# LarsELund/Bayesian-Neural-Nets

Measured on AMD Instinct MI355X. Metric: ELBO forward samples/sec, 784-1200^2-10 MNF MLP, batch 4096 per GPU, higher is better.
Workload: dtype f16 (row-scaled fp16 hi + lo split of the f32 operands: 3 mean + 1 variance MFMA products, f32 accumulate)

## Files before the change

bayesian-neural-nets_amd/csrc/gemm_common.h:

```cpp
#pragma once
#include <cstdlib>
#include <hip/hip_runtime.h>
#include <stdint.h>

namespace {

__device__ __forceinline__ void tile_of_block(int& ox, int& by, int extra_rows = 0) {
    const int nx = gridDim.x, ny = gridDim.y - extra_rows, n = nx * ny;
    int t = blockIdx.y * nx + blockIdx.x;
    if ((n & 7) == 0 && (ny & 3) == 0) {
        const int xcd = t & 7, s = t >> 3, per = n >> 3, q = ny >> 2;
        const int idx = (xcd & 1) * per + s;
        ox = idx / q;
        by = (xcd >> 1) * q + idx % q;
        return;
    }
    if ((n & 7) == 0) t = (t & 7) * (n >> 3) + (t >> 3);
    ox = t % nx; by = t / nx;
}

constexpr size_t kLdsPerCU = 160 * 1024;
constexpr int kNumCU = 256;

inline size_t lds_request(size_t needed, long nblocks) {
    long r = (nblocks + kNumCU - 1) / kNumCU;
    static const char* const res_env = getenv("LBBNN_GEMM_RESIDENCY");
    if (res_env) r = atol(res_env);
    if (r < 1) r = 1;
    if (r >= 3) return needed;
    const size_t cap = kLdsPerCU / (size_t)(r + 1) + 256;
    return needed > cap ? needed : cap;
}

template <typename K, typename A>
inline int launch_one(K kernel, dim3 grid, dim3 block, size_t lds, hipStream_t s, const A& a) {
    if (lds > 64 * 1024) {
        static size_t raised = 0;
        if (lds > raised) {
            hipError_t e = hipFuncSetAttribute(reinterpret_cast<const void*>(kernel),
                                               hipFuncAttributeMaxDynamicSharedMemorySize, (int)lds);
            if (e != hipSuccess) return (int)e;
            raised = lds;
        }
    }
    hipLaunchKernelGGL(kernel, grid, block, lds, s, a);
    return (int)hipGetLastError();
}


}
```

bayesian-neural-nets_amd/csrc/lrt_gemm_f16.hip:

```cpp
#include <cstdlib>
#include "lbbnn_device.h"
#include "lbbnn_internal.h"
#include "kl_piggy.h"
#include "gemm_common.h"
#include "../../include/lbbnn.h"

namespace {

using namespace lbbnn;
typedef float floatx4 __attribute__((ext_vector_type(4)));
typedef float floatx2 __attribute__((ext_vector_type(2)));
typedef _Float16 f16x8 __attribute__((ext_vector_type(8)));
typedef _Float16 f16x2 __attribute__((ext_vector_type(2)));

constexpr int BKS = 32;
constexpr float kS2 = 0.00390625f;
constexpr float kS2inv = 256.f;

__device__ __forceinline__ int swzx(int r) { return (((r >> 1) & 3) << 1) | ((r >> 3) & 1); }
__device__ __forceinline__ int swz4(int rowgrp) { return (0x78 >> (2 * (rowgrp & 3))) & 3; }

struct G16Args {
    const char* x; const char* e_w; const char* var_w;
    const float* mean_scale; const float* wvar_scale;
    const float* bias_mean; const float* bias_var; const float* var_scale;
    const float* eps; const uint64_t* rng;
    float* out; char* out_planes; float* std_out;
    long long row_offset;
    int ldx, ld, ldo, ldp, B, I, O;
    uint32_t rng_stream;
    int relu;
    const float* h_e; const float* h_v; float* h_slab;
    int h_ld, h_C;
    FinalizePiggy fin;
};

typedef _Float16 f16x4 __attribute__((ext_vector_type(4)));
constexpr float kHeadES = 256.f, kHeadVS = 16384.f;

__device__ __forceinline__ uint32_t cvt_pk_h(float a, float b) {
    const floatx2 v = {a, b};
    return __builtin_bit_cast(uint32_t, __builtin_convertvector(v, f16x2));
}
__device__ __forceinline__ float h_lo(uint32_t p) { return (float)__builtin_bit_cast(f16x2, p)[0]; }
__device__ __forceinline__ float h_hi(uint32_t p) { return (float)__builtin_bit_cast(f16x2, p)[1]; }

struct OC16 { float bm[4], bv[4], vs[4], ms[4]; };

__device__ __forceinline__ void ld4f(const float* p, int o, int O, float fill, float out[4]) {
    if (!p) { out[0] = out[1] = out[2] = out[3] = fill; return; }
    if (o + 3 < O && ((reinterpret_cast<uintptr_t>(p + o) & 15u) == 0)) {
        const float4 t = *reinterpret_cast<const float4*>(p + o);
        out[0] = t.x; out[1] = t.y; out[2] = t.z; out[3] = t.w;
    } else {
#pragma unroll
        for (int r = 0; r < 4; ++r) out[r] = (o + r < O) ? p[o + r] : fill;
    }
}

template <int TO, int TB, int NPV>
__device__ __forceinline__ void epilogue16(const G16Args& a, int o0, int q, int lr, int brow0,
                                           const floatx4 (&accm)[TO][TB], const floatx4 (&accv)[TO][TB]) {
    const bool ovec = ((a.O & 3) == 0) && (!a.out || (((a.ldo & 3) == 0) && ((reinterpret_cast<uintptr_t>(a.out) & 15u) == 0))) &&
                      (!a.eps || (reinterpret_cast<uintptr_t>(a.eps) & 15u) == 0) &&
                      (!a.std_out || (reinterpret_cast<uintptr_t>(a.std_out) & 15u) == 0);
    uint64_t seed = 0, offs = 0;
    if (!a.eps) { seed = a.rng[0]; offs = a.rng[1]; }
    OC16 oc[TO];
#pragma unroll
    for (int i = 0; i < TO; ++i) {
        const int o = o0 + i * 16 + 4 * q;
        if (o < a.O) {
            ld4f(a.bias_mean, o, a.O, 0.f, oc[i].bm);
            ld4f(a.bias_var, o, a.O, 0.f, oc[i].bv);
            ld4f(a.var_scale, o, a.O, 1.f, oc[i].vs);
            ld4f(a.mean_scale, o, a.O, 1.f, oc[i].ms);
            float wv[4];
            ld4f(a.wvar_scale, o, a.O, 1.f, wv);
#pragma unroll
            for (int r = 0; r < 4; ++r) oc[i].vs[r] = (wv[r] * kS2inv) * oc[i].vs[r];
        }
    }
    float pe[TO][TB][4];
    if (a.eps) {
#pragma unroll
        for (int i = 0; i < TO; ++i) {
            const int o = o0 + i * 16 + 4 * q;
#pragma unroll
            for (int j = 0; j < TB; ++j) {
                const int b = brow0 + j * 16;
                if (o >= a.O || b >= a.B) continue;
                const float* p = a.eps + (size_t)b * a.O + o;
                if (ovec) { const float4 t = *reinterpret_cast<const float4*>(p); pe[i][j][0] = t.x; pe[i][j][1] = t.y; pe[i][j][2] = t.z; pe[i][j][3] = t.w; }
                else {
#pragma unroll
                    for (int r = 0; r < 4; ++r) pe[i][j][r] = (o + r < a.O) ? p[r] : 0.f;
                }
            }
        }
    }
    const bool head = a.h_slab != nullptr;
    float4 he4[TO], hv4[TO];
    if (head) {
#pragma unroll
        for (int i = 0; i < TO; ++i) {
            const int o = o0 + i * 16 + 4 * q;
            he4[i] = make_float4(0.f, 0.f, 0.f, 0.f); hv4[i] = he4[i];
            if (lr < a.h_C && o < a.O) {
                he4[i] = *reinterpret_cast<const float4*>(a.h_e + (size_t)lr * a.h_ld + o);
                hv4[i] = *reinterpret_cast<const float4*>(a.h_v + (size_t)lr * a.h_ld + o);
            }
        }
    }
    __builtin_amdgcn_sched_barrier(0);
    const bool odd = q & 1;
    floatx4 hm[TB], hv[TB];
#pragma unroll
    for (int j = 0; j < TB; ++j) { hm[j] = floatx4{0.f, 0.f, 0.f, 0.f}; hv[j] = floatx4{0.f, 0.f, 0.f, 0.f}; }
#pragma unroll
    for (int i = 0; i < TO; ++i) {
        const int o = o0 + i * 16 + 4 * q;
        const bool oin = o < a.O;
        f16x4 ehd = {0, 0, 0, 0}, eld = {0, 0, 0, 0}, vhd = {0, 0, 0, 0}, vld = {0, 0, 0, 0};
        if (head) {
            const float4 e4 = he4[i], v4 = hv4[i];
            const uint32_t eh0 = cvt_pk_h(e4.x * kHeadES, e4.y * kHeadES), eh1 = cvt_pk_h(e4.z * kHeadES, e4.w * kHeadES);
            const uint32_t el0 = cvt_pk_h(e4.x * kHeadES - h_lo(eh0), e4.y * kHeadES - h_hi(eh0));
            const uint32_t el1 = cvt_pk_h(e4.z * kHeadES - h_lo(eh1), e4.w * kHeadES - h_hi(eh1));
            const uint32_t vh0 = cvt_pk_h(v4.x * kHeadVS, v4.y * kHeadVS), vh1 = cvt_pk_h(v4.z * kHeadVS, v4.w * kHeadVS);
            ehd = __builtin_bit_cast(f16x4, make_uint2(eh0, eh1)); eld = __builtin_bit_cast(f16x4, make_uint2(el0, el1));
            vhd = __builtin_bit_cast(f16x4, make_uint2(vh0, vh1));
            if (NPV == 3) {
                const uint32_t vl0 = cvt_pk_h(v4.x * kHeadVS - h_lo(vh0), v4.y * kHeadVS - h_hi(vh0));
                const uint32_t vl1 = cvt_pk_h(v4.z * kHeadVS - h_lo(vh1), v4.w * kHeadVS - h_hi(vh1));
                vld = __builtin_bit_cast(f16x4, make_uint2(vl0, vl1));
            }
        }
#pragma unroll
        for (int j = 0; j < TB; ++j) {
            const int b = brow0 + j * 16;
            const bool live = oin && b < a.B;
            float e[4] = {0.f, 0.f, 0.f, 0.f};
            if (a.eps) {
#pragma unroll
                for (int r = 0; r < 4; ++r) e[r] = pe[i][j][r];
            } else if (live) {
                philox_normal4(seed, offs, a.rng_stream, (uint64_t)(a.row_offset + b), (uint32_t)(o >> 2), e);
            }
            float res[4], sd[4];
#pragma unroll
            for (int r = 0; r < 4; ++r) {
                sd[r] = sqrt_hw(accv[i][j][r] * oc[i].vs[r] + oc[i].bv[r]);
                const float m = accm[i][j][r] * oc[i].ms[r] + oc[i].bm[r] + sd[r] * e[r];
                res[r] = a.relu ? fmaxf(m, 0.f) : m;
            }
            if (a.out && live) {
                float* p = a.out + (size_t)b * a.ldo + o;
                if (ovec) *reinterpret_cast<float4*>(p) = make_float4(res[0], res[1], res[2], res[3]);
                else {
#pragma unroll
                    for (int r = 0; r < 4; ++r) if (o + r < a.O) p[r] = res[r];
                }
            }
            if (a.std_out && live) {
                float* p = a.std_out + (size_t)b * a.O + o;
                if (ovec) *reinterpret_cast<float4*>(p) = make_float4(sd[0], sd[1], sd[2], sd[3]);
                else {
#pragma unroll
                    for (int r = 0; r < 4; ++r) if (o + r < a.O) p[r] = sd[r];
                }
            }
            if (head) {
                float hx[4];
#pragma unroll
                for (int r = 0; r < 4; ++r) hx[r] = (live && o + r < a.O) ? res[r] : 0.f;
                const uint32_t h01 = cvt_pk_h(hx[0], hx[1]), h23 = cvt_pk_h(hx[2], hx[3]);
                const uint32_t l01 = cvt_pk_h(hx[0] - h_lo(h01), hx[1] - h_hi(h01)), l23 = cvt_pk_h(hx[2] - h_lo(h23), hx[3] - h_hi(h23));
                const f16x4 xh = __builtin_bit_cast(f16x4, make_uint2(h01, h23)), xl = __builtin_bit_cast(f16x4, make_uint2(l01, l23));
                const float s0 = hx[0] * hx[0] * kS2, s1 = hx[1] * hx[1] * kS2, s2 = hx[2] * hx[2] * kS2, s3 = hx[3] * hx[3] * kS2;
                const uint32_t q01 = cvt_pk_h(s0, s1), q23 = cvt_pk_h(s2, s3);
                const f16x4 sh = __builtin_bit_cast(f16x4, make_uint2(q01, q23));
                hm[j] = __builtin_amdgcn_mfma_f32_16x16x16f16(ehd, xh, hm[j], 0, 0, 0);
                hm[j] = __builtin_amdgcn_mfma_f32_16x16x16f16(eld, xh, hm[j], 0, 0, 0);
                hm[j] = __builtin_amdgcn_mfma_f32_16x16x16f16(ehd, xl, hm[j], 0, 0, 0);
                hv[j] = __builtin_amdgcn_mfma_f32_16x16x16f16(vhd, sh, hv[j], 0, 0, 0);
                if (NPV == 3) {
                    const uint32_t r01 = cvt_pk_h(s0 - h_lo(q01), s1 - h_hi(q01)), r23 = cvt_pk_h(s2 - h_lo(q23), s3 - h_hi(q23));
                    const f16x4 sl = __builtin_bit_cast(f16x4, make_uint2(r01, r23));
                    hv[j] = __builtin_amdgcn_mfma_f32_16x16x16f16(vld, sh, hv[j], 0, 0, 0);
                    hv[j] = __builtin_amdgcn_mfma_f32_16x16x16f16(vhd, sl, hv[j], 0, 0, 0);
                }
            }
            if (a.out_planes) {
                const uint32_t h01 = cvt_pk_h(res[0], res[1]), h23 = cvt_pk_h(res[2], res[3]);
                const uint32_t l01 = cvt_pk_h(res[0] - h_lo(h01), res[1] - h_hi(h01));
                const uint32_t l23 = cvt_pk_h(res[2] - h_lo(h23), res[3] - h_hi(h23));
                const auto s0 = __builtin_amdgcn_permlane16_swap(h01, l01, false, false);
                const auto s1 = __builtin_amdgcn_permlane16_swap(h23, l23, false, false);
                if (live) {
                    const int kk = o & ~7;
                    char* p = a.out_planes + (size_t)b * a.ldp * 4 + (size_t)(kk >> 5) * 128 + ((kk >> 3) & 3) * 32 + (odd ? 16 : 0);
                    *reinterpret_cast<uint4*>(p) = make_uint4(s0[0], s1[0], s0[1], s1[1]);
                }
            }
        }
    }
    if (head) {
        const int ot = o0 / (TO * 16);
#pragma unroll
        for (int j = 0; j < TB; ++j) {
            const int b = brow0 + j * 16;
            if (b < a.B) {
                float* p = a.h_slab + ((size_t)ot * a.B + b) * 32 + 4 * q;
                *reinterpret_cast<float4*>(p) = make_float4(hm[j][0], hm[j][1], hm[j][2], hm[j][3]);
                *reinterpret_cast<float4*>(p + 16) = make_float4(hv[j][0], hv[j][1], hv[j][2], hv[j][3]);
            }
        }
    }
}

template <int TO, int TB, int WB, int NPV, bool XPL>
__device__ __forceinline__ void gemm_f16s_body(const G16Args& a) {
    static_assert(NPV == 1 || NPV == 3, "one or three variance products");
    constexpr int BN = TO * 16, BM = TB * WB * 16;
    constexpr int VROW = NPV == 1 ? 64 : 128;
    constexpr int XB = BM * 128, WRB = BN * 128, VRB = BN * VROW, BUFB = XB + WRB + VRB;
    constexpr int NGX = BM / 8, NGW = BN / 8, NGV = VRB / 1024, NG = NGX + NGW + NGV, NPW = (NG + WB - 1) / WB;
    static_assert(VRB % 1024 == 0, "whole 1-KiB pieces");
    extern __shared__ __attribute__((aligned(16))) char smc[];

    const int tid = threadIdx.x, lane = tid & 63;
    const int wv = __builtin_amdgcn_readfirstlane(tid >> 6);
    const int lr = lane & 15, q = lane >> 4;
    if (a.fin.n > 0 && blockIdx.y == gridDim.y - 1) {
        if (blockIdx.x == 0) kl_finalize_piggy<WB>(kernarg_as<G16Args>()->fin, reinterpret_cast<float*>(smc));
        return;
    }
    int tox, tby;
    tile_of_block(tox, tby, a.fin.n > 0 ? 1 : 0);
    const int o0 = tox * BN, b0 = tby * BM;

    const size_t xsz = XPL ? (size_t)a.B * a.ldx * 4 : ((size_t)(a.B - 1) * a.ldx + a.I) * 4;
    const unsigned xbytes = (unsigned)min((size_t)0x7FFFFFF0u, xsz);
    const unsigned wbytes = (unsigned)min((size_t)0x7FFFFFF0u, (size_t)a.O * a.ld * 4);
    const __amdgpu_buffer_rsrc_t rx = __builtin_amdgcn_make_buffer_rsrc((void*)a.x, 0, (int)xbytes, 0x00020000);
    const __amdgpu_buffer_rsrc_t re = __builtin_amdgcn_make_buffer_rsrc((void*)a.e_w, 0, (int)wbytes, 0x00020000);
    const __amdgpu_buffer_rsrc_t rv = __builtin_amdgcn_make_buffer_rsrc((void*)a.var_w, 0, (int)(NPV == 1 ? wbytes / 2 : wbytes), 0x00020000);
    int gv[NPW], kx[NPW];
#pragma unroll
    for (int u = 0; u < NPW; ++u) {
        const int g = wv + WB * u;
        if (g < NGX) {
            const int row = 8 * g + (lane >> 3);
            const int slot = (lane & 7) ^ swzx(row & 15);
            gv[u] = (int)((size_t)min(b0 + row, a.B - 1) * a.ldx * 4) + 16 * slot;
            kx[u] = XPL ? -1 : 4 * slot;
        } else if (g < NGX + NGW || NPV == 3) {
            const int gw = g - NGX, row = 8 * (gw % NGW) + (lane >> 3);
            const int slot = (lane & 7) ^ swzx(row & 15);
            gv[u] = (int)((size_t)min(o0 + row, a.O - 1) * a.ld * 4) + 16 * slot;
            kx[u] = -1;
        } else {
            const int gw = g - NGX - NGW, row = 16 * gw + (lane >> 2);
            const int slot = (lane & 3) ^ swz4(row >> 2);
            gv[u] = (int)((size_t)min(o0 + row, a.O - 1) * a.ld * 2) + 16 * slot;
            kx[u] = -1;
        }
    }
    const int nsteps = (a.I + BKS - 1) / BKS;
    const bool has_tail = !XPL && (a.I % BKS) != 0;
    int gvt[NPW];
#pragma unroll
    for (int u = 0; u < NPW; ++u)
        gvt[u] = (kx[u] >= 0 && (nsteps - 1) * BKS + kx[u] >= a.I) ? 0x7FFFFFF0 : gv[u];
    auto dma_pieces = [&](int c, char* buf, const int (&va)[NPW]) {
#pragma unroll
        for (int u = 0; u < NPW; ++u) {
            const int g = wv + WB * u;
            if (g < NG) {
                const int loff = g < NGX ? g * 1024 : XB + (g - NGX) * 1024;
                auto* dst = (__attribute__((address_space(3))) void*)(buf + loff);
                if (g < NGX)                 __builtin_amdgcn_raw_ptr_buffer_load_lds(rx, dst, 16, va[u], c * 128, 0, 0);
                else if (g - NGX < NGW)      __builtin_amdgcn_raw_ptr_buffer_load_lds(re, dst, 16, va[u], c * 128, 0, 0);
                else                         __builtin_amdgcn_raw_ptr_buffer_load_lds(rv, dst, 16, va[u], c * VROW, 0, 0);
            }
        }
    };
    auto dma_step = [&](int c, char* buf) {
        if (has_tail && c == nsteps - 1) dma_pieces(c, buf, gvt);
        else dma_pieces(c, buf, gv);
    };

    floatx4 accm[TO][TB], accv[TO][TB];
#pragma unroll
    for (int i = 0; i < TO; ++i)
#pragma unroll
        for (int j = 0; j < TB; ++j) { accm[i][j] = floatx4{0.f, 0.f, 0.f, 0.f}; accv[i][j] = floatx4{0.f, 0.f, 0.f, 0.f}; }

    const int gx = swzx(lr);
    const int xo0 = (wv * TB * 16 + lr) * 128 + 16 * ((2 * q) ^ gx);
    const int xo1 = (wv * TB * 16 + lr) * 128 + 16 * ((2 * q + 1) ^ gx);
    const int woh = XB + lr * 128 + 16 * ((2 * q) ^ gx);
    const int wol = XB + lr * 128 + 16 * ((2 * q + 1) ^ gx);
    const int vo1 = XB + WRB + lr * 64 + 16 * (q ^ swz4(lr >> 2));

    uint4 xu[TB][2];
    uint4 eh[TO], el[TO], vh[TO], vl[TO];
    auto read_frags = [&](const char* cur) {
#pragma unroll
        for (int j = 0; j < TB; ++j) {
            xu[j][0] = *reinterpret_cast<const uint4*>(cur + xo0 + j * 16 * 128);
            xu[j][1] = *reinterpret_cast<const uint4*>(cur + xo1 + j * 16 * 128);
        }
#pragma unroll
        for (int i = 0; i < TO; ++i) {
            eh[i] = *reinterpret_cast<const uint4*>(cur + woh + i * 16 * 128);
            el[i] = *reinterpret_cast<const uint4*>(cur + wol + i * 16 * 128);
            if (NPV == 3) {
                vh[i] = *reinterpret_cast<const uint4*>(cur + WRB + woh + i * 16 * 128);
                vl[i] = *reinterpret_cast<const uint4*>(cur + WRB + wol + i * 16 * 128);
            } else {
                vh[i] = *reinterpret_cast<const uint4*>(cur + vo1 + i * 16 * 64);
            }
        }
    };
    auto mfmas = [&]() {
        f16x8 xh[TB], xl[TB], sh[TB], sl[TB];
#pragma unroll
        for (int j = 0; j < TB; ++j) {
            if (XPL) {
                xh[j] = __builtin_bit_cast(f16x8, xu[j][0]);
                xl[j] = __builtin_bit_cast(f16x8, xu[j][1]);
                if (NPV == 1) {
                    const f16x8 pa = xh[j] * (_Float16)0.0625f, pb = xl[j] * (_Float16)0.125f;
                    const f16x8 t = pa * pb;
                    sh[j] = pa * pa + t;
                } else {
                    uint32_t ph[4], pl[4];
#pragma unroll
                    for (int t = 0; t < 4; ++t) {
                        const float h0 = (float)xh[j][2 * t], h1 = (float)xh[j][2 * t + 1];
                        const float l0 = (float)xl[j][2 * t], l1 = (float)xl[j][2 * t + 1];
                        const float s0 = (h0 * h0 + 2.f * h0 * l0) * kS2, s1 = (h1 * h1 + 2.f * h1 * l1) * kS2;
                        ph[t] = cvt_pk_h(s0, s1);
                        pl[t] = cvt_pk_h(s0 - h_lo(ph[t]), s1 - h_hi(ph[t]));
                    }
                    sh[j] = __builtin_bit_cast(f16x8, make_uint4(ph[0], ph[1], ph[2], ph[3]));
                    sl[j] = __builtin_bit_cast(f16x8, make_uint4(pl[0], pl[1], pl[2], pl[3]));
                }
            } else {
                const float4 f0 = __builtin_bit_cast(float4, xu[j][0]), f1 = __builtin_bit_cast(float4, xu[j][1]);
                const float v[8] = {f0.x, f0.y, f0.z, f0.w, f1.x, f1.y, f1.z, f1.w};
                uint32_t ph[4], pl[4], qh[4] = {0, 0, 0, 0}, ql[4] = {0, 0, 0, 0};
#pragma unroll
                for (int t = 0; t < 4; ++t) {
                    const float v0 = v[2 * t], v1 = v[2 * t + 1];
                    ph[t] = cvt_pk_h(v0, v1);
                    pl[t] = cvt_pk_h(v0 - h_lo(ph[t]), v1 - h_hi(ph[t]));
                    if (NPV == 3) {
                        const float s0 = (v0 * v0) * kS2, s1 = (v1 * v1) * kS2;
                        qh[t] = cvt_pk_h(s0, s1);
                        ql[t] = cvt_pk_h(s0 - h_lo(qh[t]), s1 - h_hi(qh[t]));
                    }
                }
                xh[j] = __builtin_bit_cast(f16x8, make_uint4(ph[0], ph[1], ph[2], ph[3]));
                xl[j] = __builtin_bit_cast(f16x8, make_uint4(pl[0], pl[1], pl[2], pl[3]));
                if (NPV == 1) {
                    const f16x8 pa = xh[j] * (_Float16)0.0625f, pb = xl[j] * (_Float16)0.125f;
                    const f16x8 t2 = pa * pb;
                    sh[j] = pa * pa + t2;
                } else {
                    sh[j] = __builtin_bit_cast(f16x8, make_uint4(qh[0], qh[1], qh[2], qh[3]));
                }
                sl[j] = __builtin_bit_cast(f16x8, make_uint4(ql[0], ql[1], ql[2], ql[3]));
            }
        }
#pragma unroll
        for (int j = 0; j < TB; ++j) {
#pragma unroll
            for (int i = 0; i < TO; ++i) {
                const f16x8 ah = __builtin_bit_cast(f16x8, eh[i]), al = __builtin_bit_cast(f16x8, el[i]);
                accm[i][j] = __builtin_amdgcn_mfma_f32_16x16x32_f16(ah, xh[j], accm[i][j], 0, 0, 0);
                accm[i][j] = __builtin_amdgcn_mfma_f32_16x16x32_f16(al, xh[j], accm[i][j], 0, 0, 0);
                accm[i][j] = __builtin_amdgcn_mfma_f32_16x16x32_f16(ah, xl[j], accm[i][j], 0, 0, 0);
                const f16x8 bh = __builtin_bit_cast(f16x8, vh[i]);
                accv[i][j] = __builtin_amdgcn_mfma_f32_16x16x32_f16(bh, sh[j], accv[i][j], 0, 0, 0);
                if (NPV == 3) {
                    accv[i][j] = __builtin_amdgcn_mfma_f32_16x16x32_f16(__builtin_bit_cast(f16x8, vl[i]), sh[j], accv[i][j], 0, 0, 0);
                    accv[i][j] = __builtin_amdgcn_mfma_f32_16x16x32_f16(bh, sl[j], accv[i][j], 0, 0, 0);
                }
            }
        }
    };

    dma_step(0, smc);
    __syncthreads();
    for (int c = 0; c < nsteps; ++c) {
        read_frags(smc + (c & 1) * BUFB);
        __builtin_amdgcn_sched_barrier(0);
        if (c + 1 < nsteps) dma_step(c + 1, smc + ((c & 1) ^ 1) * BUFB);
        __builtin_amdgcn_sched_barrier(0);
        mfmas();
        __builtin_amdgcn_sched_barrier(0);
        __syncthreads();
    }
    epilogue16<TO, TB, NPV>(a, o0, q, lr, b0 + wv * TB * 16 + lr, accm, accv);
}

template <int TO, int TB, int WB, int NPV, bool XPL>
__global__ __launch_bounds__(WB * 64, 2) void lrt_gemm_f16s_kernel(const G16Args a) {
    gemm_f16s_body<TO, TB, WB, NPV, XPL>(a);
}

template <int TO, int TB, int WB>
int launch16(G16Args& a, int npv, bool xpl, hipStream_t s, bool* hosted) {
    constexpr int BN = TO * 16, BM = TB * WB * 16;
    dim3 grid((a.O + BN - 1) / BN, (a.B + BM - 1) / BM, 1), block(WB * 64);
    const long nblocks = (long)grid.x * grid.y;
    const size_t lds = lds_request(2u * (BM * 128 + BN * 128 + BN * (npv == 1 ? 64 : 128)), nblocks);
    const int fin_n = a.fin.n;
    a.fin.n = 0;
    if (fin_n > 0 && hosted) {
        a.fin.n = fin_n;
        if (piggy_lds_bytes(a.fin) <= lds) { grid.y += 1; *hosted = true; }
        else a.fin.n = 0;
    }
    if (npv == 1) {
        if (xpl) return launch_one(lrt_gemm_f16s_kernel<TO, TB, WB, 1, true>, grid, block, lds, s, a);
        return launch_one(lrt_gemm_f16s_kernel<TO, TB, WB, 1, false>, grid, block, lds, s, a);
    }
    if (xpl) return launch_one(lrt_gemm_f16s_kernel<TO, TB, WB, 3, true>, grid, block, lds, s, a);
    return launch_one(lrt_gemm_f16s_kernel<TO, TB, WB, 3, false>, grid, block, lds, s, a);
}

__global__ __launch_bounds__(256) void format_x_kernel(const FormatJob j) {
    format_x_items(j, (size_t)blockIdx.x * 256 + threadIdx.x, (size_t)gridDim.x * 256);
}

struct HeadFinArgs {
    const float* slab; const float* bias_mean; const float* bias_var; const float* eps; const uint64_t* rng;
    float* out; long long row_offset;
    int n_ot, B, C, ldo, log_softmax; uint32_t rng_stream;
};

__global__ __launch_bounds__(256) void head_finalize_kernel(const HeadFinArgs a) {
    const int t = blockIdx.x * 256 + threadIdx.x, b = t >> 4, q = (t >> 2) & 3, g = t & 3;
    const bool rowok = b < a.B;
    float m[4] = {0.f, 0.f, 0.f, 0.f}, v[4] = {0.f, 0.f, 0.f, 0.f};
    if (rowok) {
        float4 pm[4], pv[4];
#pragma unroll
        for (int k = 0; k < 4; ++k) {
            const int ot = g + 4 * k;
            pm[k] = make_float4(0.f, 0.f, 0.f, 0.f); pv[k] = pm[k];
            if (ot < a.n_ot) {
                const float* p = a.slab + ((size_t)ot * a.B + b) * 32 + 4 * q;
                pm[k] = *reinterpret_cast<const float4*>(p); pv[k] = *reinterpret_cast<const float4*>(p + 16);
            }
        }
        for (int ot = g + 16; ot < a.n_ot; ot += 4) {
            const float* p = a.slab + ((size_t)ot * a.B + b) * 32 + 4 * q;
            const float4 xm = *reinterpret_cast<const float4*>(p), xv = *reinterpret_cast<const float4*>(p + 16);
            pm[0].x += xm.x; pm[0].y += xm.y; pm[0].z += xm.z; pm[0].w += xm.w;
            pv[0].x += xv.x; pv[0].y += xv.y; pv[0].z += xv.z; pv[0].w += xv.w;
        }
        m[0] = (pm[0].x + pm[1].x) + (pm[2].x + pm[3].x); m[1] = (pm[0].y + pm[1].y) + (pm[2].y + pm[3].y);
        m[2] = (pm[0].z + pm[1].z) + (pm[2].z + pm[3].z); m[3] = (pm[0].w + pm[1].w) + (pm[2].w + pm[3].w);
        v[0] = (pv[0].x + pv[1].x) + (pv[2].x + pv[3].x); v[1] = (pv[0].y + pv[1].y) + (pv[2].y + pv[3].y);
        v[2] = (pv[0].z + pv[1].z) + (pv[2].z + pv[3].z); v[3] = (pv[0].w + pv[1].w) + (pv[2].w + pv[3].w);
    }
#pragma unroll
    for (int r = 0; r < 4; ++r) {
        m[r] += dpp_get<0xB1>(m[r]); m[r] += dpp_get<0x4E>(m[r]);
        v[r] += dpp_get<0xB1>(v[r]); v[r] += dpp_get<0x4E>(v[r]);
    }
    float e[4] = {0.f, 0.f, 0.f, 0.f};
    const int c0 = 4 * q;
    if (rowok && c0 < a.C) {
        if (a.eps) {
#pragma unroll
            for (int r = 0; r < 4; ++r) if (c0 + r < a.C) e[r] = a.eps[(size_t)b * a.C + c0 + r];
        } else {
            philox_normal4(a.rng[0], a.rng[1], a.rng_stream, (uint64_t)(a.row_offset + b), (uint32_t)q, e);
        }
    }
    float res[4];
    float mx = -INFINITY;
#pragma unroll
    for (int r = 0; r < 4; ++r) {
        const int c = c0 + r;
        const bool in = rowok && c < a.C;
        const float bm = (in && a.bias_mean) ? a.bias_mean[c] : 0.f, bv = (in && a.bias_var) ? a.bias_var[c] : 0.f;
        const float sd = sqrt_hw(v[r] * (kS2inv / kHeadVS) + bv);
        res[r] = m[r] * (1.f / kHeadES) + bm + sd * e[r];
        if (in) mx = fmaxf(mx, res[r]);
    }
    if (a.log_softmax) {
        mx = fmaxf(mx, dpp_get<0x141>(mx));
        mx = fmaxf(mx, dpp_get<0x140>(mx));
        float se = 0.f;
#pragma unroll
        for (int r = 0; r < 4; ++r) if (rowok && c0 + r < a.C) se += expf(res[r] - mx);
        se += dpp_get<0x141>(se);
        se += dpp_get<0x140>(se);
        const float lse = mx + logf(se);
#pragma unroll
        for (int r = 0; r < 4; ++r) res[r] -= lse;
    }
    if (rowok && g == 0)
#pragma unroll
        for (int r = 0; r < 4; ++r) if (c0 + r < a.C) a.out[(size_t)b * a.ldo + c0 + r] = res[r];
}

}

extern "C" int64_t lbbnn_head_slab_floats(int B, int O) {
    if (B <= 0 || O <= 0) return 0;
    return (int64_t)((O + 79) / 80) * B * 32;
}

extern "C" int lbbnn_format_x(const float* x, int ldx, void* planes, int ldp, int B, int I, void* stream) {
    if (B == 0) return 0;
    if (!x || !planes) return LBBNN_E_NULL;
    if (B < 0 || I <= 0 || ldx < I || ldp < I) return LBBNN_E_SHAPE;
    if ((I & 7) || (ldx & 3) || (ldp & 31) || (reinterpret_cast<uintptr_t>(x) & 15u) || (reinterpret_cast<uintptr_t>(planes) & 15u))
        return LBBNN_E_ALIGN;
    const size_t n = (size_t)B * (ldp >> 3);
    const int blocks = (int)min((size_t)2048, (n + 255) / 256);
    const FormatJob j{x, static_cast<char*>(planes), ldx, ldp, B, I};
    hipLaunchKernelGGL(format_x_kernel, dim3(blocks), dim3(256), 0, static_cast<hipStream_t>(stream), j);
    return (int)hipGetLastError();
}

extern "C" int lbbnn_lrt_gemm_ex(const lbbnn_gemm_desc_t* d, void* stream) {
    if (!d) return LBBNN_E_NULL;
    const int B = d->B, I = d->I, O = d->O, flags = d->flags;
    if (flags & ~(LBBNN_F_RELU | LBBNN_F_F16S | LBBNN_F_VAR1 | LBBNN_F_XPLANES)) return LBBNN_E_FLAGS;
    if (!(flags & LBBNN_F_F16S)) return LBBNN_E_FLAGS;
    if (B == 0 && I > 0 && O > 0 && d->n_layers == 0 && !d->advance) return 0;
    if (!d->x || !d->e_w || !d->var_w || !d->mean_scale || !d->wvar_scale) return LBBNN_E_NULL;
    if (!d->eps && !d->rng) return LBBNN_E_NOISE;
    if (B <= 0 || I <= 0 || O <= 16 || d->ldx < I || (d->out && d->ldo < O)) return LBBNN_E_SHAPE;
    const bool xpl = (flags & LBBNN_F_XPLANES) != 0;
    if (d->ld < I || (d->ld & 31) || (I & 7)) return LBBNN_E_ALIGN;
    if ((I % BKS) != 0 && (d->ld - I) < 8) return LBBNN_E_ALIGN;
    if ((reinterpret_cast<uintptr_t>(d->e_w) | reinterpret_cast<uintptr_t>(d->var_w) | reinterpret_cast<uintptr_t>(d->x)) & 15u) return LBBNN_E_ALIGN;
    if (xpl ? (d->ldx & 31) != 0 : (d->ldx & 3) != 0) return LBBNN_E_ALIGN;
    if (d->out_planes && ((O & 7) || (d->ldp & 31) || d->ldp < O || (reinterpret_cast<uintptr_t>(d->out_planes) & 15u))) return LBBNN_E_ALIGN;
    if ((size_t)B * d->ldx * 4 >= 0x7FFFFFF0u || (size_t)O * d->ld * 4 >= 0x7FFFFFF0u) return LBBNN_E_SHAPE;
    if (d->n_layers < 0 || (d->n_layers > 0 && !d->layers) || (d->advance && !d->rng_live)) return LBBNN_E_NULL;
    const bool head = d->head_out != nullptr;
    if (head) {
        if (!d->head_e || !d->head_v || !d->head_slab) return LBBNN_E_NULL;
        if (d->head_classes <= 0 || d->head_classes > 16 || d->head_ld < O || (d->head_ld & 3) || d->head_ldo < d->head_classes) return LBBNN_E_SHAPE;
        if ((O & 3) || ((reinterpret_cast<uintptr_t>(d->head_e) | reinterpret_cast<uintptr_t>(d->head_v) | reinterpret_cast<uintptr_t>(d->head_slab)) & 15u)) return LBBNN_E_ALIGN;
        if (!d->head_eps && !d->rng) return LBBNN_E_NOISE;
        if (!(flags & LBBNN_F_RELU)) return LBBNN_E_FLAGS;
    } else if (!d->out && !d->out_planes) return LBBNN_E_NULL;

    G16Args a;
    a.x = static_cast<const char*>(d->x); a.e_w = static_cast<const char*>(d->e_w); a.var_w = static_cast<const char*>(d->var_w);
    a.mean_scale = d->mean_scale; a.wvar_scale = d->wvar_scale;
    a.bias_mean = d->bias_mean; a.bias_var = d->bias_var; a.var_scale = d->var_scale;
    a.eps = d->eps; a.rng = d->rng; a.out = d->out; a.out_planes = static_cast<char*>(d->out_planes); a.std_out = d->std_out;
    a.row_offset = d->row_offset; a.ldx = d->ldx; a.ld = d->ld; a.ldo = d->ldo; a.ldp = d->ldp; a.B = B; a.I = I; a.O = O;
    a.rng_stream = d->rng_stream; a.relu = (flags & LBBNN_F_RELU) ? 1 : 0;
    a.h_e = head ? d->head_e : nullptr; a.h_v = head ? d->head_v : nullptr; a.h_slab = head ? d->head_slab : nullptr;
    a.h_ld = d->head_ld; a.h_C = d->head_classes;
    a.fin = FinalizePiggy{};
    const bool want_fin = d->n_layers > 0 || d->advance;
    if (d->n_layers > 0) {
        if (const int rc = fill_finalize_args(d->layers, d->n_layers, d->fin_rng, a.fin.l, a.fin.active)) return rc;
        if (d->kl_total) for (int i = 0; i < d->n_layers; ++i) if (!a.fin.active[i]) return LBBNN_E_NULL;
        a.fin.n = d->n_layers; a.fin.total = d->kl_total;
        a.fin.rng_adv = d->advance ? d->rng_live : nullptr; a.fin.adv = d->advance;
    }
    hipStream_t s = static_cast<hipStream_t>(stream);
    const int npv = (flags & LBBNN_F_VAR1) ? 1 : 3;
    bool hosted = false;
    const long blocks_big = (long)((O + 79) / 80) * ((B + 127) / 128);
    int rc;
    if (blocks_big >= 256 && B >= 96) rc = launch16<5, 2, 4>(a, npv, xpl, s, &hosted);
    else rc = launch16<5, 1, 2>(a, npv, xpl, s, &hosted);
    if (rc) return rc;
    if (head) {
        HeadFinArgs h;
        h.slab = d->head_slab; h.bias_mean = d->head_bias_mean; h.bias_var = d->head_bias_var; h.eps = d->head_eps; h.rng = d->rng;
        h.out = d->head_out; h.row_offset = d->row_offset; h.n_ot = (O + 79) / 80; h.B = B; h.C = d->head_classes; h.ldo = d->head_ldo;
        h.log_softmax = (d->head_flags & LBBNN_F_LOG_SOFTMAX) ? 1 : 0; h.rng_stream = d->head_rng_stream;
        hipLaunchKernelGGL(head_finalize_kernel, dim3((16 * (size_t)B + 255) / 256), dim3(256), 0, s, h);
        rc = (int)hipGetLastError();
        if (rc) return rc;
    }
    if (!want_fin || hosted) return rc;
    if (d->n_layers > 0)
        return launch_kl_finalize_all(a.fin.l, a.fin.active, d->n_layers, d->advance ? d->rng_live : nullptr, d->advance,
                                      d->kl_total, s);
    return lbbnn_rng_advance(d->rng_live, d->advance, stream);
}
```

Measured before the change: 32.40 million.

## Stage epilogue constants in LDS and precompute Philox noise during prologue

The per-feature bias/scale vectors and head fp16 hi/lo splits are now loaded once per block by one thread per feature during the last K-step and written to the idle LDS buffer, instead of every lane redundantly loading and converting them in the epilogue. Several Philox normal draws are computed right after the first DMA issue so they overlap with memory latency rather than sitting on the epilogue's critical path. Grid tile dimensions are passed as kernel arguments. This adds LDS traffic and extra registers held through the main loop for the precomputed noise, which may lower occupancy.

Result: faster. 33.55 million, median of 6 (+3.5%).

```diff
diff --git a/bayesian-neural-nets_amd/csrc/gemm_common.h b/bayesian-neural-nets_amd/csrc/gemm_common.h
--- a/bayesian-neural-nets_amd/csrc/gemm_common.h
+++ b/bayesian-neural-nets_amd/csrc/gemm_common.h
@@ -5,8 +5,8 @@
 
 namespace {
 
-__device__ __forceinline__ void tile_of_block(int& ox, int& by, int extra_rows = 0) {
-    const int nx = gridDim.x, ny = gridDim.y - extra_rows, n = nx * ny;
+__device__ __forceinline__ void tile_of_block(int& ox, int& by, int nx, int ny) {
+    const int n = nx * ny;
     int t = blockIdx.y * nx + blockIdx.x;
     if ((n & 7) == 0 && (ny & 3) == 0) {
         const int xcd = t & 7, s = t >> 3, per = n >> 3, q = ny >> 2;
@@ -17,6 +17,9 @@
     }
     if ((n & 7) == 0) t = (t & 7) * (n >> 3) + (t >> 3);
     ox = t % nx; by = t / nx;
+}
+__device__ __forceinline__ void tile_of_block(int& ox, int& by, int extra_rows = 0) {
+    tile_of_block(ox, by, (int)gridDim.x, (int)gridDim.y - extra_rows);
 }
 
 constexpr size_t kLdsPerCU = 160 * 1024;
diff --git a/bayesian-neural-nets_amd/csrc/lrt_gemm_f16.hip b/bayesian-neural-nets_amd/csrc/lrt_gemm_f16.hip
--- a/bayesian-neural-nets_amd/csrc/lrt_gemm_f16.hip
+++ b/bayesian-neural-nets_amd/csrc/lrt_gemm_f16.hip
@@ -32,6 +32,7 @@
     int relu;
     const float* h_e; const float* h_v; float* h_slab;
     int h_ld, h_C;
+    int gx, gy;
     FinalizePiggy fin;
 };
 
@@ -45,42 +46,87 @@
 __device__ __forceinline__ float h_lo(uint32_t p) { return (float)__builtin_bit_cast(f16x2, p)[0]; }
 __device__ __forceinline__ float h_hi(uint32_t p) { return (float)__builtin_bit_cast(f16x2, p)[1]; }
 
-struct OC16 { float bm[4], bv[4], vs[4], ms[4]; };
-
-__device__ __forceinline__ void ld4f(const float* p, int o, int O, float fill, float out[4]) {
-    if (!p) { out[0] = out[1] = out[2] = out[3] = fill; return; }
-    if (o + 3 < O && ((reinterpret_cast<uintptr_t>(p + o) & 15u) == 0)) {
-        const float4 t = *reinterpret_cast<const float4*>(p + o);
-        out[0] = t.x; out[1] = t.y; out[2] = t.z; out[3] = t.w;
-    } else {
-#pragma unroll
-        for (int r = 0; r < 4; ++r) out[r] = (o + r < O) ? p[o + r] : fill;
-    }
-}
-
-template <int TO, int TB, int NPV>
-__device__ __forceinline__ void epilogue16(const G16Args& a, int o0, int q, int lr, int brow0,
+template <int TO>
+struct EpiImage {
+    static constexpr int BN = TO * 16;
+    static constexpr int kConst = 0, kHeadE = 4 * BN * 4, kHeadV = kHeadE + TO * 64 * 16, kBytes = kHeadV + TO * 64 * 16;
+};
+
+typedef const LBBNN_CONST_AS G16Args KArgs;
+
+template <int NQ>
+struct EpiStage { float c[5]; float4 he[NQ], hv[NQ]; };
+
+__device__ __forceinline__ float ld1f(const float* p, int o, bool in, float fill) { return (p && in) ? p[o] : fill; }
+
+template <int TO, int WB>
+__device__ __forceinline__ void stage_load(const KArgs& a, int o0, int tid, EpiStage<(TO + WB - 1) / WB>& st) {
+    constexpr int BN = TO * 16, NQ = (TO + WB - 1) / WB;
+    static_assert(WB * 64 >= BN, "one thread per feature");
+    if (tid < BN) {
+        const int o = o0 + tid;
+        const bool in = o < a.O;
+        st.c[0] = ld1f(a.bias_mean, o, in, 0.f);
+        st.c[1] = ld1f(a.bias_var, o, in, 0.f);
+        st.c[2] = ld1f(a.var_scale, o, in, 1.f);
+        st.c[3] = ld1f(a.mean_scale, o, in, 1.f);
+        st.c[4] = ld1f(a.wvar_scale, o, in, 1.f);
+    }
+    if (a.h_slab) {
+#pragma unroll
+        for (int u = 0; u < NQ; ++u) {
+            const int s = tid + u * WB * 64;
+            const int o = o0 + (s >> 6) * 16 + 4 * ((s >> 4) & 3), cls = s & 15;
+            st.he[u] = make_float4(0.f, 0.f, 0.f, 0.f); st.hv[u] = st.he[u];
+            if (s < TO * 64 && cls < a.h_C && o < a.O) {
+                st.he[u] = *reinterpret_cast<const float4*>(a.h_e + (size_t)cls * a.h_ld + o);
+                st.hv[u] = *reinterpret_cast<const float4*>(a.h_v + (size_t)cls * a.h_ld + o);
+            }
+        }
+    }
+}
+
+template <int TO, int WB, int NPV>
+__device__ __forceinline__ void stage_store(const KArgs& a, int tid, const EpiStage<(TO + WB - 1) / WB>& st, char* img) {
+    constexpr int BN = TO * 16, NQ = (TO + WB - 1) / WB;
+    typedef EpiImage<TO> IM;
+    if (tid < BN) {
+        float* c = reinterpret_cast<float*>(img + IM::kConst);
+        c[tid] = st.c[0];
+        c[BN + tid] = st.c[1];
+        c[2 * BN + tid] = (st.c[4] * kS2inv) * st.c[2];
+        c[3 * BN + tid] = st.c[3];
+    }
+    if (a.h_slab) {
+#pragma unroll
+        for (int u = 0; u < NQ; ++u) {
+            const int s = tid + u * WB * 64;
+            if (s >= TO * 64) continue;
+            const float4 e4 = st.he[u], v4 = st.hv[u];
+            const uint32_t eh0 = cvt_pk_h(e4.x * kHeadES, e4.y * kHeadES), eh1 = cvt_pk_h(e4.z * kHeadES, e4.w * kHeadES);
+            const uint32_t el0 = cvt_pk_h(e4.x * kHeadES - h_lo(eh0), e4.y * kHeadES - h_hi(eh0));
+            const uint32_t el1 = cvt_pk_h(e4.z * kHeadES - h_lo(eh1), e4.w * kHeadES - h_hi(eh1));
+            const uint32_t vh0 = cvt_pk_h(v4.x * kHeadVS, v4.y * kHeadVS), vh1 = cvt_pk_h(v4.z * kHeadVS, v4.w * kHeadVS);
+            uint32_t vl0 = 0, vl1 = 0;
+            if (NPV == 3) {
+                vl0 = cvt_pk_h(v4.x * kHeadVS - h_lo(vh0), v4.y * kHeadVS - h_hi(vh0));
+                vl1 = cvt_pk_h(v4.z * kHeadVS - h_lo(vh1), v4.w * kHeadVS - h_hi(vh1));
+            }
+            reinterpret_cast<uint4*>(img + IM::kHeadE)[s] = make_uint4(eh0, eh1, el0, el1);
+            reinterpret_cast<uint4*>(img + IM::kHeadV)[s] = make_uint4(vh0, vh1, vl0, vl1);
+        }
+    }
+}
+
+template <int TO, int TB, int NPV, int NPRE>
+__device__ __forceinline__ void epilogue16(const KArgs& a, int o0, int q, int lr, int brow0, const char* img,
+                                           uint64_t seed, uint64_t offs, const float (&pre)[NPRE > 0 ? NPRE : 1][4],
                                            const floatx4 (&accm)[TO][TB], const floatx4 (&accv)[TO][TB]) {
+    typedef EpiImage<TO> IM;
+    constexpr int BN = TO * 16;
     const bool ovec = ((a.O & 3) == 0) && (!a.out || (((a.ldo & 3) == 0) && ((reinterpret_cast<uintptr_t>(a.out) & 15u) == 0))) &&
                       (!a.eps || (reinterpret_cast<uintptr_t>(a.eps) & 15u) == 0) &&
                       (!a.std_out || (reinterpret_cast<uintptr_t>(a.std_out) & 15u) == 0);
-    uint64_t seed = 0, offs = 0;
-    if (!a.eps) { seed = a.rng[0]; offs = a.rng[1]; }
-    OC16 oc[TO];
-#pragma unroll
-    for (int i = 0; i < TO; ++i) {
-        const int o = o0 + i * 16 + 4 * q;
-        if (o < a.O) {
-            ld4f(a.bias_mean, o, a.O, 0.f, oc[i].bm);
-            ld4f(a.bias_var, o, a.O, 0.f, oc[i].bv);
-            ld4f(a.var_scale, o, a.O, 1.f, oc[i].vs);
-            ld4f(a.mean_scale, o, a.O, 1.f, oc[i].ms);
-            float wv[4];
-            ld4f(a.wvar_scale, o, a.O, 1.f, wv);
-#pragma unroll
-            for (int r = 0; r < 4; ++r) oc[i].vs[r] = (wv[r] * kS2inv) * oc[i].vs[r];
-        }
-    }
     float pe[TO][TB][4];
     if (a.eps) {
 #pragma unroll
@@ -100,18 +146,7 @@
         }
     }
     const bool head = a.h_slab != nullptr;
-    float4 he4[TO], hv4[TO];
-    if (head) {
-#pragma unroll
-        for (int i = 0; i < TO; ++i) {
-            const int o = o0 + i * 16 + 4 * q;
-            he4[i] = make_float4(0.f, 0.f, 0.f, 0.f); hv4[i] = he4[i];
-            if (lr < a.h_C && o < a.O) {
-                he4[i] = *reinterpret_cast<const float4*>(a.h_e + (size_t)lr * a.h_ld + o);
-                hv4[i] = *reinterpret_cast<const float4*>(a.h_v + (size_t)lr * a.h_ld + o);
-            }
-        }
-    }
+    const float* cst = reinterpret_cast<const float*>(img + IM::kConst);
     __builtin_amdgcn_sched_barrier(0);
     const bool odd = q & 1;
     floatx4 hm[TB], hv[TB];
@@ -121,20 +156,18 @@
     for (int i = 0; i < TO; ++i) {
         const int o = o0 + i * 16 + 4 * q;
         const bool oin = o < a.O;
+        const int fo = i * 16 + 4 * q;
+        const float4 bm = *reinterpret_cast<const float4*>(cst + fo), bv = *reinterpret_cast<const float4*>(cst + BN + fo);
+        const float4 vs = *reinterpret_cast<const float4*>(cst + 2 * BN + fo), ms = *reinterpret_cast<const float4*>(cst + 3 * BN + fo);
+        const float c_bm[4] = {bm.x, bm.y, bm.z, bm.w}, c_bv[4] = {bv.x, bv.y, bv.z, bv.w};
+        const float c_vs[4] = {vs.x, vs.y, vs.z, vs.w}, c_ms[4] = {ms.x, ms.y, ms.z, ms.w};
         f16x4 ehd = {0, 0, 0, 0}, eld = {0, 0, 0, 0}, vhd = {0, 0, 0, 0}, vld = {0, 0, 0, 0};
         if (head) {
-            const float4 e4 = he4[i], v4 = hv4[i];
-            const uint32_t eh0 = cvt_pk_h(e4.x * kHeadES, e4.y * kHeadES), eh1 = cvt_pk_h(e4.z * kHeadES, e4.w * kHeadES);
-            const uint32_t el0 = cvt_pk_h(e4.x * kHeadES - h_lo(eh0), e4.y * kHeadES - h_hi(eh0));
-            const uint32_t el1 = cvt_pk_h(e4.z * kHeadES - h_lo(eh1), e4.w * kHeadES - h_hi(eh1));
-            const uint32_t vh0 = cvt_pk_h(v4.x * kHeadVS, v4.y * kHeadVS), vh1 = cvt_pk_h(v4.z * kHeadVS, v4.w * kHeadVS);
-            ehd = __builtin_bit_cast(f16x4, make_uint2(eh0, eh1)); eld = __builtin_bit_cast(f16x4, make_uint2(el0, el1));
-            vhd = __builtin_bit_cast(f16x4, make_uint2(vh0, vh1));
-            if (NPV == 3) {
-                const uint32_t vl0 = cvt_pk_h(v4.x * kHeadVS - h_lo(vh0), v4.y * kHeadVS - h_hi(vh0));
-                const uint32_t vl1 = cvt_pk_h(v4.z * kHeadVS - h_lo(vh1), v4.w * kHeadVS - h_hi(vh1));
-                vld = __builtin_bit_cast(f16x4, make_uint2(vl0, vl1));
-            }
+            const uint4 ea = reinterpret_cast<const uint4*>(img + IM::kHeadE)[i * 64 + 16 * q + lr];
+            const uint4 va = reinterpret_cast<const uint4*>(img + IM::kHeadV)[i * 64 + 16 * q + lr];
+            ehd = __builtin_bit_cast(f16x4, make_uint2(ea.x, ea.y)); eld = __builtin_bit_cast(f16x4, make_uint2(ea.z, ea.w));
+            vhd = __builtin_bit_cast(f16x4, make_uint2(va.x, va.y));
+            if (NPV == 3) vld = __builtin_bit_cast(f16x4, make_uint2(va.z, va.w));
         }
 #pragma unroll
         for (int j = 0; j < TB; ++j) {
@@ -144,14 +177,17 @@
             if (a.eps) {
 #pragma unroll
                 for (int r = 0; r < 4; ++r) e[r] = pe[i][j][r];
+            } else if (i * TB + j < NPRE) {
+#pragma unroll
+                for (int r = 0; r < 4; ++r) e[r] = pre[i * TB + j < NPRE ? i * TB + j : 0][r];
             } else if (live) {
                 philox_normal4(seed, offs, a.rng_stream, (uint64_t)(a.row_offset + b), (uint32_t)(o >> 2), e);
             }
             float res[4], sd[4];
 #pragma unroll
             for (int r = 0; r < 4; ++r) {
-                sd[r] = sqrt_hw(accv[i][j][r] * oc[i].vs[r] + oc[i].bv[r]);
-                const float m = accm[i][j][r] * oc[i].ms[r] + oc[i].bm[r] + sd[r] * e[r];
+                sd[r] = sqrt_hw(accv[i][j][r] * c_vs[r] + c_bv[r]);
+                const float m = accm[i][j][r] * c_ms[r] + c_bm[r] + sd[r] * e[r];
                 res[r] = a.relu ? fmaxf(m, 0.f) : m;
             }
             if (a.out && live) {
@@ -219,26 +255,36 @@
     }
 }
 
+#ifndef LBBNN_G16_NPRE
+#define LBBNN_G16_NPRE 4
+#endif
+constexpr int npre_of(int TO, int TB, int NPV) {
+    return NPV == 3 ? 0 : (LBBNN_G16_NPRE < TO * TB ? LBBNN_G16_NPRE : TO * TB);
+}
+
 template <int TO, int TB, int WB, int NPV, bool XPL>
 __device__ __forceinline__ void gemm_f16s_body(const G16Args& a) {
     static_assert(NPV == 1 || NPV == 3, "one or three variance products");
-    constexpr int BN = TO * 16, BM = TB * WB * 16;
+    constexpr int BN = TO * 16, BM = TB * WB * 16, NPRE = npre_of(TO, TB, NPV);
     constexpr int VROW = NPV == 1 ? 64 : 128;
     constexpr int XB = BM * 128, WRB = BN * 128, VRB = BN * VROW, BUFB = XB + WRB + VRB;
     constexpr int NGX = BM / 8, NGW = BN / 8, NGV = VRB / 1024, NG = NGX + NGW + NGV, NPW = (NG + WB - 1) / WB;
     static_assert(VRB % 1024 == 0, "whole 1-KiB pieces");
+    static_assert(EpiImage<TO>::kBytes <= BUFB, "the epilogue's operand image fits one K-step buffer");
     extern __shared__ __attribute__((aligned(16))) char smc[];
 
     const int tid = threadIdx.x, lane = tid & 63;
     const int wv = __builtin_amdgcn_readfirstlane(tid >> 6);
     const int lr = lane & 15, q = lane >> 4;
-    if (a.fin.n > 0 && blockIdx.y == gridDim.y - 1) {
+    if ((int)blockIdx.y >= a.gy) {
         if (blockIdx.x == 0) kl_finalize_piggy<WB>(kernarg_as<G16Args>()->fin, reinterpret_cast<float*>(smc));
         return;
     }
     int tox, tby;
-    tile_of_block(tox, tby, a.fin.n > 0 ? 1 : 0);
+    tile_of_block(tox, tby, a.gx, a.gy);
     const int o0 = tox * BN, b0 = tby * BM;
+    uint64_t seed = 0, offs = 0;
+    if (!a.eps) { seed = a.rng[0]; offs = a.rng[1]; }
 
     const size_t xsz = XPL ? (size_t)a.B * a.ldx * 4 : ((size_t)(a.B - 1) * a.ldx + a.I) * 4;
     const unsigned xbytes = (unsigned)min((size_t)0x7FFFFFF0u, xsz);
@@ -393,8 +439,23 @@
         }
     };
 
+    const int brow0 = b0 + wv * TB * 16 + lr;
+    float pre[NPRE > 0 ? NPRE : 1][4];
     dma_step(0, smc);
+    if (NPRE > 0) {
+        __builtin_amdgcn_sched_barrier(0);
+#pragma unroll
+        for (int t = 0; t < NPRE; ++t) {
+            const int o = o0 + (t / TB) * 16 + 4 * q, b = brow0 + (t % TB) * 16;
+            pre[t][0] = pre[t][1] = pre[t][2] = pre[t][3] = 0.f;
+            if (!a.eps && o < a.O && b < a.B)
+                philox_normal4(seed, offs, a.rng_stream, (uint64_t)(a.row_offset + b), (uint32_t)(o >> 2), pre[t]);
+        }
+        __builtin_amdgcn_sched_barrier(0);
+    }
     __syncthreads();
+    char* const img = smc + (nsteps & 1) * BUFB;
+    EpiStage<(TO + WB - 1) / WB> st;
     for (int c = 0; c < nsteps; ++c) {
         read_frags(smc + (c & 1) * BUFB);
         __builtin_amdgcn_sched_barrier(0);
@@ -402,9 +463,13 @@
         __builtin_amdgcn_sched_barrier(0);
         mfmas();
         __builtin_amdgcn_sched_barrier(0);
+        if (c + 1 == nsteps) {
+            stage_load<TO, WB>(*kernarg_as<G16Args>(), o0, tid, st);
+            stage_store<TO, WB, NPV>(*kernarg_as<G16Args>(), tid, st, img);
+        }
         __syncthreads();
     }
-    epilogue16<TO, TB, NPV>(a, o0, q, lr, b0 + wv * TB * 16 + lr, accm, accv);
+    epilogue16<TO, TB, NPV, NPRE>(*kernarg_as<G16Args>(), o0, q, lr, brow0, img, seed, offs, pre, accm, accv);
 }
 
 template <int TO, int TB, int WB, int NPV, bool XPL>
@@ -419,6 +484,7 @@
     const long nblocks = (long)grid.x * grid.y;
     const size_t lds = lds_request(2u * (BM * 128 + BN * 128 + BN * (npv == 1 ? 64 : 128)), nblocks);
     const int fin_n = a.fin.n;
+    a.gx = (int)grid.x; a.gy = (int)grid.y;
     a.fin.n = 0;
     if (fin_n > 0 && hosted) {
         a.fin.n = fin_n;
```
